# oma219/spumoni

Hardware: AMD Instinct MI355X
Metric: reads/s PML classification, 200 bp reads vs 10-hap human index (higher is better)
Workload: dtype u64

## Files before the change

### spumoni_amd/csrc/spx_cache.hip

```cpp
#include <sys/stat.h>
#include <unistd.h>
#include <algorithm>
#include <chrono>
#include <cstdio>
#include <cstring>
#include <string>
#include <thread>
#include <vector>

#include "spx_internal.h"

using namespace spx;

extern "C" {

namespace {

struct SpxFileHeader {
    char magic[8];
    char layout[56];
    uint64_t header_bytes;
    uint64_t n, r;
    uint32_t has_samples, has_docs;
    uint64_t n_text;
    uint64_t arr_bytes[spx_index::NARR];
    uint64_t arr_offset[spx_index::NARR];
    spx::DevIndex view;
    uint64_t device_bytes;
    char source_tag[128];
};

constexpr size_t STAGE = 16u << 20;

int read_to_device(FILE* f, uint64_t off, void* dst, uint64_t bytes, void* stage[2], hipStream_t st, hipEvent_t ev[2]) {
    if (fseeko(f, (off_t)off, SEEK_SET) != 0) {
        set_error("seek failed");
        return SPX_E_IO;
    }
    int b = 0;
    for (uint64_t done = 0; done < bytes; b ^= 1) {
        const size_t take = (size_t)std::min<uint64_t>(STAGE, bytes - done);
        SPX_HIP(hipEventSynchronize(ev[b]));
        if (fread(stage[b], 1, take, f) != take) {
            set_error("cache file is truncated");
            return SPX_E_IO;
        }
        SPX_HIP(hipMemcpyAsync((char*)dst + done, stage[b], take, hipMemcpyHostToDevice, st));
        SPX_HIP(hipEventRecord(ev[b], st));
        done += take;
// ... 123 lines not shown
        return SPX_E_ARG;
    }
    std::lock_guard<std::mutex> g(ix->mu);
    SPX_HIP(hipSetDevice(ix->device));
    SPX_HIP(hipDeviceSynchronize());
    SpxFileHeader h;
    memset(&h, 0, sizeof h);
    memcpy(h.magic, "SPXFLAT", 8);
    snprintf(h.layout, sizeof h.layout, "%s", SPX_LAYOUT_VERSION);
    h.header_bytes = sizeof h;
    h.n = ix->n;
    h.r = ix->r;
    h.has_samples = ix->has_samples;
    h.has_docs = ix->has_docs;
    h.n_text = ix->n_text;
    h.view = ix->view;
    {
        spx_index blank;
        blank.view = h.view;
        blank.n_text = ix->n_text;
        bind_view(&blank);
        h.view = blank.view;
    }
    h.device_bytes = ix->device_bytes;
    memcpy(h.source_tag, ix->source_tag, sizeof h.source_tag);
    uint64_t off = (sizeof h + 4095) & ~4095ull;
    for (int i = 0; i < spx_index::NARR; ++i) {
        const bool skip = i == A_FAT || i == A_FATJ;
        h.arr_bytes[i] = ix->arr_bytes[i];
        h.arr_offset[i] = skip ? 0 : off;
        if (!skip) off = (off + ix->arr_bytes[i] + 4095) & ~4095ull;
    }
    const std::string tmp = std::string(path) + ".tmp";
    FILE* f = fopen(tmp.c_str(), "wb");
    if (!f) {
        set_error("cannot create %s", tmp.c_str());
        return SPX_E_IO;
    }
    IoPool& pool = io_pool();
    std::lock_guard<std::mutex> pg(pool.mu);
    int rc = pool.init();
    if (rc == SPX_OK && (fwrite(&h, sizeof h, 1, f) != 1 || ftruncate(fileno(f), (off_t)off) != 0)) {
        set_error("write failed");
        rc = SPX_E_IO;
    }
    if (fclose(f) != 0 && rc == SPX_OK) {
        set_error("write failed (disk full?)");
        rc = SPX_E_IO;
    }
    void** arr[spx_index::NARR];
    index_arrays(ix, arr);
    for (int i = 0; i < spx_index::NARR && rc == SPX_OK; ++i)
        if (h.arr_offset[i]) rc = transfer_array(pool, tmp, h.arr_offset[i], *arr[i], h.arr_bytes[i], false, ix->device);
    if (rc == SPX_OK && rename(tmp.c_str(), path) != 0) {
        set_error("cannot rename %s to %s", tmp.c_str(), path);
        rc = SPX_E_IO;
    }
    if (rc != SPX_OK) remove(tmp.c_str());
    return rc;
}

spx_index* spx_index_load_flat(const char* path, int device) {
    if (!path) {
        set_error("path is null");
        return nullptr;
    }
    if (select_device(device) != SPX_OK) return nullptr;
    FILE* f = fopen(path, "rb");
    if (!f) {
        set_error("cannot open %s", path);
        return nullptr;
    }
    SpxFileHeader h;
    if (fread(&h, sizeof h, 1, f) != 1 || memcmp(h.magic, "SPXFLAT", 8) != 0 || h.header_bytes != sizeof h) {
        set_error("%s is not a flat-layout cache of this library", path);
        fclose(f);
        return nullptr;
    }
    h.layout[sizeof h.layout - 1] = 0;
    if (strcmp(h.layout, SPX_LAYOUT_VERSION) != 0) {
        set_error("%s was written by layout '%s', this library is '%s': rebuild the cache", path, h.layout,
                  SPX_LAYOUT_VERSION);
        fclose(f);
        return nullptr;
    }
    {
        struct stat stf;
        const uint64_t fsize = fstat(fileno(f), &stf) == 0 ? (uint64_t)stf.st_size : 0;
        const uint64_t r = h.view.r;
        const uint64_t row_bytes = h.view.compact ? sizeof(spx::Row32) : sizeof(spx::Row);
        const bool aux = h.has_samples || h.has_docs;
        uint64_t want[spx_index::NARR] = {};
        want[A_ROWS] = (r + ROW_PAD) * row_bytes;
        want[A_DIRROWS] = (r + ROW_PAD) * sizeof(spx::JumpRow);
        want[A_FAT] = (h.view.nfat + 2) * (uint64_t)h.view.fat_stride;
        want[A_FATJ] = spx::fatjs_count(h.view.nfat) * 4 + 64;
        want[A_Q] = (r + 1 + Q_PAD) * 4;
        want[A_AUX] = aux ? (r + 2) * sizeof(spx::Aux) : 0;
        want[A_SSRUN] = h.has_samples ? (r + 4) * 8 : 0;
        want[A_RUNDOCS] = h.has_docs ? (r + ROW_PAD) * 4 : 0;
        want[A_LETTERS] = 256 * sizeof(spx::LetterInfo);
        want[A_TEXT] = h.n_text ? h.n_text + 16 : 0;
        bool ok = r > 0 && r < 0xfffffff0ull && h.r > 0 && h.r <= r && h.n > 0 && h.view.n == h.n &&
                  (h.view.fat_stride == 32u || (!aux && h.view.fat_stride == 16u)) && (h.view.fat_stride == 16u || aux || h.view.compact) &&
                  (h.n_text == 0 || h.n_text + 1 == h.n || h.n_text < h.n);
        for (int i = 0; ok && i < spx_index::NARR; ++i) {
            ok = h.arr_bytes[i] == want[i];
            const bool stored = i != A_FAT && i != A_FATJ && h.arr_bytes[i] != 0;
            if (ok && stored) ok = h.arr_offset[i] >= sizeof h && h.arr_offset[i] + h.arr_bytes[i] <= fsize;
        }
        if (!ok) {
            set_error("%s: the header does not describe a consistent index (array sizes / offsets against r = %llu and the "
                      "file's %llu bytes): rebuild the cache", path, (unsigned long long)r, (unsigned long long)fsize);
            fclose(f);
            return nullptr;
        }
    }
    spx_index* ix = new spx_index();
    ix->device = device;
    h.source_tag[sizeof h.source_tag - 1] = 0;
    memcpy(ix->source_tag, h.source_tag, sizeof ix->source_tag);
    ix->n = h.n;
    ix->r = h.r;
    ix->has_samples = h.has_samples != 0;
    ix->has_docs = h.has_docs != 0;
    ix->n_text = h.n_text;
    ix->view = h.view;
    ix->device_bytes = h.device_bytes;
    const bool timing = getenv("SPX_TIMING") != nullptr;
    auto now = [] { return std::chrono::duration<double>(std::chrono::steady_clock::now().time_since_epoch()).count(); };
    auto body = [&]() -> int {
        double t0 = now();
        IoPool& pool = io_pool();
        std::lock_guard<std::mutex> pg(pool.mu);
        int rc = pool.init();
        if (rc != SPX_OK) return rc;
        if (timing) fprintf(stderr, "[spx] load_flat: staging pool %.3f s\n", now() - t0);
        void** arr[spx_index::NARR];
        index_arrays(ix, arr);
        for (int i = 0; i < spx_index::NARR; ++i) {
            ix->arr_bytes[i] = h.arr_bytes[i];
            if (h.arr_bytes[i] == 0 || h.arr_offset[i] == 0) continue;
            SPX_HIP(hipMalloc(arr[i], h.arr_bytes[i]));
            t0 = now();
            if ((rc = transfer_array(pool, path, h.arr_offset[i], *arr[i], h.arr_bytes[i], true, device)) != SPX_OK) return rc;
            if (timing) fprintf(stderr, "[spx] load_flat: array %d, %.2f GB in %.3f s\n", i, h.arr_bytes[i] / 1e9, now() - t0);
        }
        bind_view(ix);
        t0 = now();
        if ((rc = build_fat(ix)) != SPX_OK) return rc;
        if (timing) fprintf(stderr, "[spx] load_flat: fat table rebuilt in %.3f s\n", now() - t0);
        return init_runtime(ix);
    };
    const int rc = body();
    fclose(f);
    if (rc != SPX_OK) {
        spx_index_free(ix);
        return nullptr;
    }
    return ix;
}

spx_index* spx_index_clone(spx_index* src, int device) {
    if (!src) {
        set_error("index is null");
        return nullptr;
    }
    if (select_device(device) != SPX_OK) return nullptr;
    spx_index* ix = new spx_index();
    ix->device = device;
    auto body = [&]() -> int {
        std::lock_guard<std::mutex> g(src->mu);
        ix->n = src->n;
        ix->r = src->r;
// ... 44 lines not shown
        ix->force_digest_kernel = src->force_digest_kernel;
        ix->digest_parked = src->digest_parked;
        return rc;
    };
    if (body() != SPX_OK) {
        spx_index_free(ix);
        return nullptr;
    }
    return ix;
}

int spx_index_describe(const spx_index* ix, char* buf, size_t cap) {
    if (!ix || !buf || cap == 0) {
        set_error("null argument");
        return SPX_E_ARG;
    }
    const DevIndex& v = ix->view;
    char where[160] = "";
    if (getenv("SPX_DESCRIBE_ADDRESSES"))
        snprintf(where, sizeof where, ", \"rows_at\": \"%p\", \"dirrows_at\": \"%p\", \"fat_at\": \"%p\"", (void*)ix->rows, (void*)ix->dirrows, (void*)ix->fat);
    snprintf(buf, cap,
             "{\"layout\": \"%s\", \"n\": %llu, \"r\": %llu, \"flat_runs\": %u, \"letters\": %u, \"compact_rows\": %u, "
             "\"fat_slots\": %llu, \"fat_slots_per_run\": %.4f, \"fat_stride\": %u, \"has_samples\": %d, "
             "\"has_docs\": %d, \"n_text\": %llu, \"device_bytes\": %llu%s}",
             SPX_LAYOUT_VERSION, (unsigned long long)ix->n, (unsigned long long)ix->r, v.r, v.nletters, v.compact,
             (unsigned long long)v.nfat, (double)v.nfat / (double)(v.r ? v.r : 1), v.fat_stride,
             (int)ix->has_samples, (int)ix->has_docs, (unsigned long long)ix->n_text,
             (unsigned long long)(ix->device_bytes + ix->n_text), where);
    return SPX_OK;
}

}
```

### spumoni_amd/csrc/spx_flatten.hip

```cpp
#include <hipcub/hipcub.hpp>

#include <functional>

#include <algorithm>
#include <chrono>
#include <cmath>
#include <cstdio>
#include <cstdlib>
#include <vector>

#include "spx_internal.h"

namespace spx {

namespace {

constexpr int TPB = 256;
#define SPX_ALLOC0(ptr, bytes)                                   \
    do {                                                         \
        const size_t nb_ = (bytes);                              \
        SPX_HIP(hipMalloc((void**)&(ptr), nb_));                 \
        SPX_HIP(hipMemsetAsync((ptr), 0, nb_, nullptr));         \
    } while (0)
inline unsigned nblocks(uint64_t n) { return (unsigned)((n + TPB - 1) / TPB); }
// ... 277 lines not shown

__global__ void k_pack_aux(const SamplePair* samples, const uint32_t* dirdocs, uint64_t count, Aux* aux) {
    uint64_t i = blockIdx.x * (uint64_t)TPB + threadIdx.x;
    if (i >= count) return;
    const SamplePair sp = samples ? samples[i] : SamplePair{0, 0};
    aux[i] = pack_aux(sp.ss, sp.se, dirdocs ? dirdocs[i] : 0u);
}

__global__ void k_samples(const uint64_t* ssa, const uint64_t* esa, const uint32_t* Qall, uint64_t r,
                          SamplePair* out, uint64_t* ss_by_run) {
    uint64_t i = blockIdx.x * (uint64_t)TPB + threadIdx.x;
    if (i > r) return;
    SamplePair sp;
    sp.ss = i < r ? ssa[Qall[i]] : 0;
    sp.se = i > 0 ? esa[Qall[i - 1]] : 0;
    out[i] = sp;
    if (i < r) ss_by_run[i] = ssa[i];
    if (i == r) {
        ss_by_run[r] = 0;
        ss_by_run[r + 1] = 0;
    }
}

}

int build_fat(spx_index* ix) {
    hipStream_t st = nullptr;
    const uint64_t r = ix->view.r, nfat = ix->view.nfat;
    const uint32_t fat_stride = ix->view.fat_stride;
    std::vector<LetterInfo> hl(256);
    SPX_HIP(hipMemcpy(hl.data(), ix->letters, 256 * sizeof(LetterInfo), hipMemcpyDeviceToHost));
    std::vector<uint8_t> lets;
    uint64_t most_runs = 0;
    for (int c = 0; c < 256; ++c)
        if (hl[c].qend > hl[c].qbeg) {
            lets.push_back((uint8_t)c);
            most_runs = std::max<uint64_t>(most_runs, hl[c].qend - hl[c].qbeg);
            if ((hl[c].fbase & (FJ_GROUP - 1)) != 0 || hl[c].fbase + letter_slots((uint32_t)r, hl[c].bmul) > nfat) {
                set_error("index letters describe a fat table that does not fit its %llu slots", (unsigned long long)nfat);
                return SPX_E_FORMAT;
            }
        }
    if (lets.empty()) {
        set_error("index without letters");
        return SPX_E_FORMAT;
    }
// ... 468 lines not shown
    }
    if (docs) {
        SPX_HIP(hipMemcpyAsync(&last_de, d_de + (r - 1), 8, hipMemcpyDeviceToHost, st));
        SPX_HIP(hipMemcpyAsync(&first_ds, d_ds, 8, hipMemcpyDeviceToHost, st));
    }
    const bool has_ms = d_ssa && d_esa;
    SPX_HIP(hipStreamSynchronize(st));
    for (DevBuf* t : {&samples_tmp, &dirdocs_tmp, &Qall, &S, &Hs, &H, &tmp}) {
        if (t->p) (void)hipFree(t->p);
        t->p = nullptr;
    }
    if (release_inputs) release_inputs();
    size_t mem_free = 0, mem_total = 0;
    SPX_HIP(hipMemGetInfo(&mem_free, &mem_total));
    const uint32_t fat_row_bytes = sizeof(FatRow);
    const bool want_lrow = getenv("SPX_FAT_LROW") != nullptr && atoi(getenv("SPX_FAT_LROW")) != 0;
    const bool lrow = want_lrow && compact && !(has_ms || docs);
    const uint32_t fat_stride = fat_row_bytes + ((has_ms || docs || lrow) ? (uint32_t)sizeof(Aux) : 0);
    const double per_slot = fat_stride + 4.0 / FJ_GROUP ;
    const double fixed = (double)r * ((double)row_bytes + 32 + 4 + ((has_ms || docs) ? 16 : 0) + (has_ms ? 8 : 0) + (docs ? 4 : 0));
    const double to_come = (double)(64 << 20);
    double budget = 0.75 * (double)mem_total;
    if (const char* e = getenv("SPX_INDEX_BUDGET_GB")) budget = atof(e) * 1e9;
    double fat_bytes = budget - fixed;
    const double fat_bytes_free = 0.92 * (double)mem_free - to_come;
    if (fat_bytes > fat_bytes_free) fat_bytes = fat_bytes_free;
    double max_slots = fat_bytes > 0 ? fat_bytes / per_slot : 0;
    if (max_slots > 16.0 * (double)r) max_slots = 16.0 * (double)r;
    if (const char* e = getenv("SPX_FAT_SLOTS_PER_RUN")) max_slots = atof(e) * (double)r;
    double alpha = 0.7;
    if (const char* e = getenv("SPX_FAT_ALPHA")) alpha = atof(e);
    int force_bshift = -1;
    if (const char* e = getenv("SPX_FAT_BSHIFT")) {
        force_bshift = atoi(e) & 31;
        if (force_bshift > 20) force_bshift = 20;
    }
    auto geometry = [&](double K, bool commit) -> double {
        uint64_t slots = 0;
        for (uint8_t c : lets) {
            LetterInfo& li = hl[c];
            double B = force_bshift >= 0 ? (double)(1u << force_bshift)
                                         : K * pow((double)(li.qend - li.qbeg) / (double)r, -alpha);
            if (B < 1.0) B = 1.0;
            const double m = 4294967296.0 / B;
            const uint32_t bmul = m >= 4294967295.0 ? 0xffffffffu : (m < 1.0 ? 1u : (uint32_t)m);
            if (commit) {
                li.bmul = bmul;
                li.fbase = slots;
// ... 51 lines not shown
    ix->arr_bytes[A_DIRROWS] = (r + ROW_PAD) * sizeof(JumpRow);
    ix->arr_bytes[A_FAT] = (nfat + 2) * (uint64_t)fat_stride;
    ix->arr_bytes[A_FATJ] = fatjs_count(nfat) * 4 + 64;
    ix->arr_bytes[A_Q] = (r + 1 + Q_PAD) * 4;
    ix->arr_bytes[A_AUX] = ix->aux ? (r + 2) * sizeof(Aux) : 0;
    ix->arr_bytes[A_SSRUN] = ix->ss_by_run ? (r + 4) * 8 : 0;
    ix->arr_bytes[A_RUNDOCS] = ix->rundocs ? (r + ROW_PAD) * 4 : 0;
    ix->arr_bytes[A_LETTERS] = 256 * sizeof(LetterInfo);
    ix->arr_bytes[A_TEXT] = 0;
    v.n = n;
    v.r = (uint32_t)r;
    v.compact = (uint32_t)compact;
    v.nletters = nletters;
    v.nfat = nfat;
    v.init_k = (uint32_t)(r - 1);
    v.init_off = last_len - 1;
    memset(&v.init_row, 0, sizeof v.init_row);
    SPX_HIP(hipMemcpy(&v.init_row, reinterpret_cast<const char*>(ix->rows) + (r - 1) * row_bytes, row_bytes,
                      hipMemcpyDeviceToHost));
    v.init_sample = ix->has_samples ? (last_esa + 1) % n : 0;
    v.init_doc = (uint32_t)last_de;
    v.doc_at0 = (uint32_t)first_ds;
    ix->device_bytes = bytes;
    return SPX_OK;
}

}
```

### spumoni_amd/csrc/spx_internal.h

```cpp
#pragma once
#include <hip/hip_runtime.h>

#include <memory>
#include <functional>
#include <mutex>
#include <string>

#include "../../include/spumoni_gpu.h"
#include "spx_layout.h"

namespace spx {

void set_error(const char* fmt, ...);
int hip_fail(hipError_t e, const char* what, const char* file, int line);
int select_device(int device);

#define SPX_HIP(call)                                                        \
    do {                                                                     \
        hipError_t e_ = (call);                                              \
        if (e_ != hipSuccess) return spx::hip_fail(e_, #call, __FILE__, __LINE__); \
    } while (0)

struct QuietOnError {
    hipStream_t st;
// ... 75 lines not shown
    uint32_t* out_lengths;
    uint64_t* out_pointers;
    uint32_t* out_docs;
    spx_class* out_class;
    uint64_t bin_width;
    uint64_t bin_magic;
    uint64_t max_value_thr;
    WalkCounters* counters;
    uint32_t lanes_per_wave;
    uint32_t narrow;
    ChunkArgs ch;
    const uint32_t* only_flagged;
    const uint64_t* in_starts;
    uint64_t* len_mask;
    unsigned long long* claim;
    uint64_t len_mask_pairs;
};

}

namespace spx {
struct ArrayOwner {
    int device = 0;
    void* p[10] = {};
    ~ArrayOwner() {
        (void)hipSetDevice(device);
        for (void* a : p)
            if (a) (void)hipFree(a);
    }
};
}

struct spx_index {
    int device = 0;
    uint64_t n = 0, r = 0;
    bool has_samples = false, has_docs = false;
    spx::Row* rows = nullptr;
    uint32_t* q_alloc = nullptr;
    spx::JumpRow* dirrows = nullptr;
    char* fat = nullptr;
    uint32_t* fat_js = nullptr;
    spx::Aux* aux = nullptr;
    uint64_t* ss_by_run = nullptr;
    uint32_t* rundocs = nullptr;
    spx::LetterInfo* letters = nullptr;
    uint8_t* text = nullptr;
    uint64_t n_text = 0;
    static constexpr int NARR = 10;
    uint64_t arr_bytes[NARR] = {};
    std::shared_ptr<spx::ArrayOwner> owner;
    hipStream_t ctx_stream = nullptr;
    static constexpr int NDIGSCR = 15;
    hipEvent_t ev_dig = nullptr;
    hipStream_t dig_stream = nullptr;
    bool dig_used = false;
    spx::DevIndex view{};
    spx::WalkCounters* counters = nullptr;
    bool claim_used = false;
    hipEvent_t ev0 = nullptr, ev1 = nullptr, ev_done = nullptr;
    bool have_timing = false;
    hipStream_t last_stream = nullptr;
    uint64_t device_bytes = 0;
    int waves_per_cu = 0;
    int occ_blocks[8] = {};
    int num_cus = 0;
    int force_lanes_per_wave = 0;
    int force_digest_kernel = 0;
    int digest_parked = 0;
    uint8_t charhash[4] = {0, 0, 0, 0};
    char source_tag[128] = {0};
    static constexpr int PIPE_CHUNKS = 10;
// ... 41 lines not shown
           M_OUT_DOCS, M_COUNT };
    Scratch mems_scr[M_COUNT];
    hipEvent_t ev_m[4] = {nullptr, nullptr, nullptr, nullptr};
    hipStream_t mems_stream = nullptr;
    bool have_mems = false, mems_pending = false, mems_ready = false, mems_ready_docs = false;
    uint64_t mems_capacity = 0, mems_ready_n = 0;
    uint64_t mems_acc[4] = {};
    float mems_ms = 0;
    uint64_t text_bytes[3] = {0, 0, 0};
    uint64_t text_nreads = 0;
    bool text_ready = false;
    spx_class* text_cls_host = nullptr;
    int blocking_sync = 0;
    hipEvent_t ev_wait = nullptr;
    uint64_t* h_pub = nullptr;
    uint64_t* h_pub_dev = nullptr;
    int chunk_mode = 0;
    int chunk_shift = 0;
    int chunk_len = 0;
    uint64_t last_chunk_len = 0, last_chunk_bound = 0;
};

namespace spx {
enum { A_ROWS, A_DIRROWS, A_FAT, A_FATJ, A_Q, A_AUX, A_SSRUN, A_RUNDOCS, A_LETTERS, A_TEXT };
inline void index_arrays(spx_index* ix, void*** out) {
    out[A_ROWS] = (void**)&ix->rows;
    out[A_DIRROWS] = (void**)&ix->dirrows;
    out[A_FAT] = (void**)&ix->fat;
    out[A_FATJ] = (void**)&ix->fat_js;
    out[A_Q] = (void**)&ix->q_alloc;
    out[A_AUX] = (void**)&ix->aux;
    out[A_SSRUN] = (void**)&ix->ss_by_run;
    out[A_RUNDOCS] = (void**)&ix->rundocs;
    out[A_LETTERS] = (void**)&ix->letters;
    out[A_TEXT] = (void**)&ix->text;
}
inline void bind_view(spx_index* ix) {
    DevIndex& v = ix->view;
    v.rows = ix->rows;
    v.dirrows = ix->dirrows;
    v.fat = ix->fat;
    v.Q = ix->q_alloc ? ix->q_alloc + 1 : nullptr;
    v.aux = ix->aux;
    v.ss_by_run = ix->ss_by_run;
    v.rundocs = ix->rundocs;
    v.fat_js = ix->fat_js;
    v.letters = ix->letters;
    v.text = ix->text;
    v.n_text = ix->n_text;
}
int ctx_stream_of(spx_index* ix, hipStream_t* out);
int ctx_wait(spx_index* ix, hipStream_t st);
int init_runtime(spx_index* ix);
void release_votes(spx_index* ix);
void release_mems(spx_index* ix);
int build_fat(spx_index* ix);
int launch_text_check(spx_index* ix, unsigned long long* d_bad, hipStream_t stream);
int launch_text_from_index(spx_index* ix, uint8_t* d_text, uint64_t n_text, unsigned long long* d_stuck, hipStream_t stream);
int flatten_on_device(spx_index* ix, const uint8_t* d_heads, const uint64_t* d_lens,
                      const uint64_t* d_thr, const uint64_t* d_ssa, const uint64_t* d_esa,
                      const uint64_t* d_ds, const uint64_t* d_de, const std::function<void()>& release_inputs = {});
int launch_walk(spx_index* ix, int mode, const BatchArgs& args, uint64_t total_chars,
                hipStream_t stream, bool* wrote_lengths = nullptr);
int launch_ms_extend(spx_index* ix, const BatchArgs& args, hipStream_t stream);
int prepare_len_mask(spx_index* ix, int mode, BatchArgs& args);
inline uint64_t len_mask_pairs(uint64_t chars, uint64_t reads) { return (chars >> 7) + reads + 2; }
int launch_len_expand(spx_index* ix, const BatchArgs& args, hipStream_t stream);
int launch_walk_chunked(spx_index* ix, int mode, const BatchArgs& args, uint64_t total_chars, hipStream_t stream,
                        bool* done, uint64_t geom_chars = 0);
int launch_text_count(const void* d_vals, int value_bytes, const uint64_t* d_offs, const uint32_t* d_gap, uint64_t nreads,
                      uint64_t* d_line_bytes, uint64_t* d_line_start, void* d_cub, size_t cub_bytes, hipStream_t st);
size_t text_scan_bytes(uint64_t nreads);
int launch_text_write(const void* d_vals, int value_bytes, const uint64_t* d_offs, const uint32_t* d_gap, uint64_t nreads,
                      const uint64_t* d_line_start, char* d_text, hipStream_t st);
int launch_digest(spx_index* ix, int kind, uint32_t k, uint32_t w, const uint8_t* d_seqs, const uint64_t* d_offs,
                  uint64_t nreads, uint64_t total_chars, uint8_t* d_out, uint64_t* d_out_offs, hipStream_t stream,
                  bool* parked = nullptr);
}
```

### spumoni_amd/csrc/spx_layout.h

```cpp
#pragma once
#include <stdint.h>

#if defined(__HIPCC__)
#define SPX_HD __host__ __device__ __forceinline__
#else
#define SPX_HD inline
#endif

#define SPX_LAYOUT_VERSION "spx-flat-r06a"

namespace spx {

constexpr uint64_t MASK40 = (1ull << 40) - 1;
constexpr uint32_t NO_LETTER = 0xffffffffu;
constexpr int ROW_PAD = 8;
constexpr int Q_PAD = 16;

struct alignas(16) Row {
    uint64_t q0;
    uint64_t q1;
};
constexpr uint32_t ROOM_SAT = 127;

SPX_HD Row pack_row(uint32_t H, uint64_t len, uint32_t LFrun, uint64_t LFoff, bool thr_ok, uint64_t room) {
    Row r;
    const uint64_t rm = room < ROOM_SAT ? room : ROOM_SAT;
    r.q0 = (len & MASK40) | ((uint64_t)(H & 0xff) << 40) | ((uint64_t)(LFrun & 0xffff) << 48);
    r.q1 = (LFoff & MASK40) | ((uint64_t)(LFrun >> 16) << 40) | ((uint64_t)(thr_ok ? 1 : 0) << 56) | (rm << 57);
    return r;
}
SPX_HD uint32_t row_room(const Row& r) { return (uint32_t)(r.q1 >> 57); }
SPX_HD uint64_t row_len(const Row& r) { return r.q0 & MASK40; }
// ... 98 lines not shown
    uint64_t fbase;
};
SPX_HD uint32_t fat_block(uint32_t k, uint32_t bmul) { return (uint32_t)(((uint64_t)k * bmul) >> 32); }
SPX_HD uint64_t letter_slots(uint32_t r, uint32_t bmul) { return ((uint64_t)fat_block(r, bmul) + 2 + 7) & ~7ull; }

struct alignas(16) Aux {
    uint64_t a0, a1;
};
SPX_HD Aux pack_aux(uint64_t ss, uint64_t se, uint32_t docs) {
    Aux a;
    a.a0 = (ss & MASK40) | ((se & 0xffffff) << 40);
    a.a1 = ((se >> 24) & 0xffff) | ((uint64_t)docs << 16);
    return a;
}
SPX_HD uint64_t aux_ss(const Aux& a) { return a.a0 & MASK40; }
SPX_HD uint64_t aux_se(const Aux& a) { return (a.a0 >> 40) | ((a.a1 & 0xffff) << 24); }
SPX_HD uint32_t aux_docs(const Aux& a) { return (uint32_t)(a.a1 >> 16); }

struct SamplePair {
    uint64_t ss;
    uint64_t se;
};

struct DevIndex {
    const Row* rows;
    const JumpRow* dirrows;
    const char* fat;
    const uint32_t* Q;
    const Aux* aux;
    const uint64_t* ss_by_run;
    const uint32_t* rundocs;
    const uint32_t* fat_js;
    uint32_t fat_stride;
    const LetterInfo* letters;
    const uint8_t* text;
    uint64_t n_text;
    uint64_t n;
    uint32_t r;
    uint32_t compact;
    uint32_t nletters;
    uint64_t nfat;
    uint32_t init_k;
    uint64_t init_off;
    Row32 init_row;
    uint64_t init_sample;
    uint32_t init_doc;
    uint32_t doc_at0;
};

SPX_HD const Row& row_at(const DevIndex& ix, uint64_t k) {
    return *reinterpret_cast<const Row*>(reinterpret_cast<const char*>(ix.rows) + k * (ix.compact ? sizeof(Row32) : sizeof(Row)));
}

constexpr uint64_t PIECE_MAX = 65535;

SPX_HD uint64_t run_of_position(const uint64_t* S, uint64_t r, uint64_t p) {
    uint64_t lo = 0, hi = r;
    while (hi - lo > 1) {
        const uint64_t mid = lo + (hi - lo) / 2;
        if (S[mid] <= p)
            lo = mid;
        else
            hi = mid;
    }
    return lo;
}

template <class F>
SPX_HD uint32_t for_each_piece(uint64_t len, uint64_t lf, const uint64_t* S, uint64_t a, uint64_t nb, uint32_t span, F&& f) {
    uint32_t np = 0;
// ... 19 lines not shown
```

### spumoni_amd/csrc/spx_walk_fast.inc

```

enum : uint32_t { Q_LAND = 0, Q_FAT = 1, Q_STEP = 2, Q_READ = 3, Q_CHARS = 4, Q_FATJ = 5, Q_QS = 6, Q_DIR = 7, Q_DONE = 8, Q_SAMP = 9, Q_START = 10, Q_WANT = 11 };
enum : uint32_t {
    F_EMB = 1,
    F_NOROW = 2,
    F_QUIRK = 4,
    F_WIDE = 16,
    F_FADD = 32,
    F_HAVEC = 64,
    F_SAMPD = 128
};
enum : uint32_t { A_STEP = 1, A_EMIT = 2, A_DECIDE = 4 };
#ifndef SPX_STEP_REPS
#define SPX_STEP_REPS 2
#endif
constexpr int STEP_REPS = SPX_STEP_REPS;
constexpr uint32_t OFF_LAST32 = 0xffffffffu;
#ifndef SPX_CHUNK_CLAIM
#define SPX_CHUNK_CLAIM 64
#endif
constexpr uint32_t CHUNK_CLAIM = SPX_CHUNK_CLAIM;
static_assert(CHUNK_CLAIM >= 64, "a claim covers at least one iteration's worst case: 64 lanes ending a read each");

__device__ __forceinline__ uint32_t dpp_swap1(uint32_t v) { return (uint32_t)__builtin_amdgcn_mov_dpp((int)v, 0xB1, 0xf, 0xf, true); }

struct alignas(16) HotLetter {
    uint32_t bmul;
    uint32_t present;
    uint64_t fat0;
};

__device__ __forceinline__ void lf_target_ct(uint32_t LFrun, uint32_t LFoff, uint32_t cums, uint32_t off, uint32_t& k0,
                                             uint32_t& offp, uint32_t& t_out) {
    lf_target_c(LFrun, LFoff, cums, off, k0, offp);
    const uint32_t t = k0 - LFrun;
    t_out = (t < 4 && off <= 126) ? t : 4u;
}

template <int MODE, bool DOC, bool NARROW, int CHUNK = 0, bool EARLY = false, bool DYN = false>
__global__ void __launch_bounds__(WALK_TPB) k_walk_fast(const DevIndex ix, const BatchArgs b) {
    constexpr bool AUX = (MODE == SPX_MODE_MS) || DOC;
    constexpr bool PML = MODE == SPX_MODE_PML;
    if (CHUNK == 2 && b.ch.round > 1 && b.ch.pending[b.ch.round] == 0) return;
    __shared__ HotLetter s_hot[256];
#ifndef SPX_PGRP
#define SPX_PGRP 16
#endif
    constexpr int PGRP = SPX_PGRP, PROW = WALK_TPB + 1;
    constexpr int PLPG = PGRP / 2, PNG = 64 / PLPG;
    __shared__ uint64_t s_ptrs[MODE == SPX_MODE_MS && CHUNK != 2 ? PGRP * PROW : 1];
    constexpr bool DSTAGE = PML && DOC && CHUNK != 2;
    constexpr int DGRP = 32, DROW = DGRP + 2;
    __shared__ uint16_t s_docs[DSTAGE ? WALK_TPB * DROW : 1];
    const LetterInfo* const s_let = ix.letters;
    __shared__ uint32_t s_win[8 * WALK_TPB];
    const char* const rows_b = reinterpret_cast<const char*>(ix.rows);
    const char* const fat_b = reinterpret_cast<const char*>(ix.fat);
    const uint32_t fs = ix.fat_stride;
    const bool lrow = !AUX && fs == 32 && ix.aux == nullptr;
    for (int t = threadIdx.x; t < 256; t += blockDim.x) {
        const LetterInfo li = ix.letters[t];
        s_hot[t] = HotLetter{li.bmul, li.qbeg != li.qend ? 1u : 0u, (uint64_t)(uintptr_t)(fat_b + li.fbase * fs)};
    }
    __syncthreads();
    const char* const dir_b = reinterpret_cast<const char*>(ix.dirrows);
    const char* const fatj_b = reinterpret_cast<const char*>(ix.fat_js);
    const char* const q_b = reinterpret_cast<const char*>(ix.Q);
    const char* const seq_b = reinterpret_cast<const char*>(b.seqs);
    const char* const off_b = reinterpret_cast<const char*>(b.offs);
    const uint32_t R = ix.r;
    const uint32_t fs_shift = fs == 32 ? 5 : 4;
    const bool want_class = PML && CHUNK == 0 && b.out_class != nullptr;
    const bool want_len = PML && CHUNK != 2 && b.out_lengths != nullptr;
    const uint32_t lpw = b.lanes_per_wave;
    const uint32_t nlanes = (uint32_t)((((uint64_t)gridDim.x * blockDim.x) >> 6) * lpw);
    const uint32_t nitems = CHUNK ? (uint32_t)*b.ch.nchunks : (uint32_t)b.nreads;
    const uint64_t ch_org = CHUNK ? b.offs[0] : 0;
    uint8_t* const ch_flags = CHUNK ? b.ch.flags - (ch_org & ~7ull) : nullptr;
    WalkState* const ch_ckpt = CHUNK ? b.ch.ckpt - (ch_org >> CKPT_SHIFT) : nullptr;
    const char* const item_b = CHUNK ? reinterpret_cast<const char*>(b.ch.desc) : off_b;
    constexpr uint32_t ITEM_BYTES = CHUNK ? sizeof(ChunkDesc) : 8;
    const uint32_t tid = threadIdx.x;
    static_assert(!DYN || (CHUNK == 0 && !EARLY), "only the plain, full launch deals its reads on demand");
    uint32_t w_n0 = 0, w_e0 = 0, w_n1 = 0, w_e1 = 0;
    bool w_pend = false;
// ... 65 lines not shown
                const u32x4 t = *(GV16)(uintptr_t)a2;
                r2x = t.x, r2y = t.y, r2z = t.z, r2w = t.w;
            }
            ga = V16{odd ? r2x : r1x, odd ? r2y : r1y, odd ? r2z : r1z, odd ? r2w : r1w};
            const uint32_t zx = dpp_swap1(odd ? r1x : r2x), zy = dpp_swap1(odd ? r1y : r2y), zz = dpp_swap1(odd ? r1z : r2z),
                           zw = dpp_swap1(odd ? r1w : r2w);
            gb = V16{w_own ? zx : 0u, w_own ? zy : 0u, w_own ? zz : 0u, w_own ? zw : 0u};
        }
        side_doc = 0;
        side_aux = Aux{0, 0};
        side_in = 0;
        claimed = 0;
        if (CHUNK == 0 && b.in_starts != nullptr && ph == Q_READ) side_in = b.in_starts[rd];
        if (DOC && ph == Q_SAMP) side_doc = ix.rundocs[k];
        if (AUX && ph == Q_DIR) side_aux = ix.aux[length];
        if (DYN && w_pend && (tid & 63) == 0) claimed = atomicAdd(b.claim, (unsigned long long)CHUNK_CLAIM);
    };
    if (EARLY) issue_gather();
    while (__builtin_amdgcn_ballot_w64(ph != Q_DONE) != 0) {
        if (!EARLY) issue_gather();
        uint32_t act = 0, hd = 0;
        uint32_t rflag = 0;
        bool pred_ev = false;
        uint32_t d_trun = 0, d_toff = 0, d_srun = 0, d_soff = 0, d_bits = 0;
        Aux d_aux{0, 0};
        bool d_lrow = false;
        uint64_t fbits = 0;
        uint32_t fxi = 0;
        bool flush = false;
        bool pflush = false, pheld = false, pheld_end = false;
        uint32_t pfxi = 0;
        uint64_t phold = 0;
        COUNT(w_rows, ph == Q_LAND);
        COUNT(w_dir, ph == Q_FAT || (ph >= Q_FATJ && ph <= Q_DIR));

        if (ph == Q_LAND) {
            const uint32_t len = ga.x & 0xffffu;
            const uint32_t o = off == OFF_LAST32 ? len - 1 : off;
            if (o >= len) {
                off = o - len;
                k++;
                addr += sizeof(Row32);
            } else {
                off = o;
                q0 = u64of(ga.x, ga.y);
                q1 = u64of(ga.z, ga.w);
                fl = (fl & ~F_NOROW) | F_EMB;
                act = A_STEP;
            }
        } else if (ph == Q_FAT) {
            const uint32_t hq = ga.x;
            const uint32_t w1l = ga.z, w1h = ga.w;
            const bool nosucc = (w1h >> 29) & 1, esc = (w1h >> 30) & 1;
            const bool quirk = fl & F_QUIRK;
            const bool found = nosucc || hq > k || (quirk && hq == k);
            if (found && !esc && !quirk) {
                d_trun = hq - (w1l & 0x7ffffu);
// ... 63 lines not shown
                        bin_lo = (nb - 1) * w;
                        bin_max = above = below = 0;
                        sum_max = 0;
                    }
                    act = A_STEP;
                    if (CHUNK == 2) {
                        ph = Q_START;
                        addr = reinterpret_cast<const char*>(b.ch.round > 1 ? b.ch.reentry + rd : b.ch.ends + rd + 1);
                        fl = F_WIDE;
                        act = 0;
                    }
                }
            } else if (ph == Q_CHARS) {
                s_win[0 * WALK_TPB + tid] = ga.x;
                s_win[1 * WALK_TPB + tid] = ga.y;
                s_win[2 * WALK_TPB + tid] = ga.z;
                s_win[3 * WALK_TPB + tid] = ga.w;
                s_win[4 * WALK_TPB + tid] = gb.x;
                s_win[5 * WALK_TPB + tid] = gb.y;
                s_win[6 * WALK_TPB + tid] = gb.z;
                s_win[7 * WALK_TPB + tid] = gb.w;
                ph = Q_STEP;
                act = A_STEP;
            } else if (CHUNK == 2 && ph == Q_START) {
                k = ga.x;
                length = ga.y;
                {
                    const uint64_t offp = u64of(ga.z, ga.w);
                    off = offp == OFF_END ? OFF_LAST32 : (uint32_t)offp;
                }
                sample = u64of(gb.x, gb.y);
                doc = gb.z;
                tlimit = b.ch.round > 1 ? gb.w : 0xffffffffu;
                ph = Q_LAND;
                addr = rows_b + (uint64_t)k * sizeof(Row32);
                fl = F_WIDE;
                {
                    const char* const cp = reinterpret_cast<const char*>(ch_ckpt + ((base + m - 1) >> CKPT_SHIFT));
                    cka = *reinterpret_cast<const V16*>(cp);
                    ckb = *reinterpret_cast<const V16*>(cp + 16);
                }
            } else if (ph == Q_FATJ) {
                const uint32_t lo = (length & 2) ? ga.z : ga.x, hi = (length & 2) ? ga.w : ga.y;
                length = (length & 1) ? hi : lo;
                fl |= F_WIDE;
                ph = Q_QS;
// ... 36 lines not shown
                    if (AUX) {
                        const Aux a = ix.aux[jdir + ((below_thr && off > 0) ? 1u : 0u)];
                        if (MODE == SPX_MODE_MS) sample = below_thr ? aux_se(a) : aux_ss(a);
                        if (DOC) doc = below_thr ? (aux_docs(a) >> 16) : (aux_docs(a) & 0xffffu);
                    }
                    if (!below_thr) {
                        k = LFrun_k;
                        off = LFoff_k + off;
                    } else if (off > 0) {
                        k = LFrun_k;
                        off = LFoff_k + off - 1;
                    } else {
                        if (jdir <= qbeg) atomicAdd(&b.counters->error, 1ull);
                        const bool ps = jr_psame(e);
                        const uint32_t srun = jr_sLFrun(e);
                        k = ps ? srun : srun - 1;
                        off = ps ? (uint32_t)jr_sLFoff(e) - 1 : OFF_LAST32;
                    }
                    length = 0;
                    fl &= ~(F_EMB | F_QUIRK);
                    rflag = 3;
                    act = A_EMIT;
                }
            }
        }
        if (AUX && ph == Q_SAMP) {
            if (MODE == SPX_MODE_MS) sample = u64of(ga.x, ga.y);
            if (DOC) doc = side_doc & 0xffffu;
            fl |= F_SAMPD;
            ph = Q_STEP;
            act = A_STEP;
        }

        {
            const bool dec = act & A_DECIDE;
            const bool nosucc = (d_bits >> 9) & 1, psame = (d_bits >> 8) & 1;
            const bool below_thr = nosucc || (k < d_trun) || (k == d_trun && off < d_toff);
            COUNT(w_pred, (dec && below_thr) || pred_ev);
            if (dec) {
                if (below_thr && ((d_bits >> 10) & 1)) atomicAdd(&b.counters->error, 1ull);
                const bool last = below_thr && !psame;
                k = d_srun - (last ? 1u : 0u);
                off = last ? OFF_LAST32 : d_soff - (below_thr ? 1u : 0u);
                hd = last ? ((d_bits >> 16) & 0xffu) : (d_bits & 0xffu);
                if (MODE == SPX_MODE_MS) sample = below_thr ? aux_se(d_aux) : aux_ss(d_aux);
                if (DOC) doc = below_thr ? (aux_docs(d_aux) >> 16) : (aux_docs(d_aux) & 0xffffu);
// ... 437 lines not shown
```

Before: 1.098 billion.

## Add precomputed start table to skip first backward-search steps per read

Builds a device table of walk states for every string of the first `depth` letters, filled level by level with a GPU kernel. When a read's last `depth` characters are all present letters, the PML walk fetches one table entry and replays the stored reset bits into the match-length and bin statistics, instead of doing `depth` LF/jump steps. The table is sized against the memory budget and takes space from the fat table. It is rebuilt at cache load rather than stored in the file, which bumps the layout version. Saving is at most a few steps out of roughly 200 per read, and the new phase adds a dependent load plus extra branching and ballots in the hot loop.

```diff
diff --git a/spumoni_amd/csrc/spx_cache.hip b/spumoni_amd/csrc/spx_cache.hip
--- a/spumoni_amd/csrc/spx_cache.hip
+++ b/spumoni_amd/csrc/spx_cache.hip
@@ -23,8 +23,8 @@
     uint64_t n, r;
     uint32_t has_samples, has_docs;
     uint64_t n_text;
-    uint64_t arr_bytes[spx_index::NARR];
-    uint64_t arr_offset[spx_index::NARR];
+    uint64_t arr_bytes[spx_index::NFILE];
+    uint64_t arr_offset[spx_index::NFILE];
     spx::DevIndex view;
     uint64_t device_bytes;
     char source_tag[128];
@@ -194,10 +194,10 @@
         bind_view(&blank);
         h.view = blank.view;
     }
-    h.device_bytes = ix->device_bytes;
+    h.device_bytes = ix->device_bytes - ix->arr_bytes[A_START];
     memcpy(h.source_tag, ix->source_tag, sizeof h.source_tag);
     uint64_t off = (sizeof h + 4095) & ~4095ull;
-    for (int i = 0; i < spx_index::NARR; ++i) {
+    for (int i = 0; i < spx_index::NFILE; ++i) {
         const bool skip = i == A_FAT || i == A_FATJ;
         h.arr_bytes[i] = ix->arr_bytes[i];
         h.arr_offset[i] = skip ? 0 : off;
@@ -222,7 +222,7 @@
     }
     void** arr[spx_index::NARR];
     index_arrays(ix, arr);
-    for (int i = 0; i < spx_index::NARR && rc == SPX_OK; ++i)
+    for (int i = 0; i < spx_index::NFILE && rc == SPX_OK; ++i)
         if (h.arr_offset[i]) rc = transfer_array(pool, tmp, h.arr_offset[i], *arr[i], h.arr_bytes[i], false, ix->device);
     if (rc == SPX_OK && rename(tmp.c_str(), path) != 0) {
         set_error("cannot rename %s to %s", tmp.c_str(), path);
@@ -262,7 +262,7 @@
         const uint64_t r = h.view.r;
         const uint64_t row_bytes = h.view.compact ? sizeof(spx::Row32) : sizeof(spx::Row);
         const bool aux = h.has_samples || h.has_docs;
-        uint64_t want[spx_index::NARR] = {};
+        uint64_t want[spx_index::NFILE] = {};
         want[A_ROWS] = (r + ROW_PAD) * row_bytes;
         want[A_DIRROWS] = (r + ROW_PAD) * sizeof(spx::JumpRow);
         want[A_FAT] = (h.view.nfat + 2) * (uint64_t)h.view.fat_stride;
@@ -276,7 +276,7 @@
         bool ok = r > 0 && r < 0xfffffff0ull && h.r > 0 && h.r <= r && h.n > 0 && h.view.n == h.n &&
                   (h.view.fat_stride == 32u || (!aux && h.view.fat_stride == 16u)) && (h.view.fat_stride == 16u || aux || h.view.compact) &&
                   (h.n_text == 0 || h.n_text + 1 == h.n || h.n_text < h.n);
-        for (int i = 0; ok && i < spx_index::NARR; ++i) {
+        for (int i = 0; ok && i < spx_index::NFILE; ++i) {
             ok = h.arr_bytes[i] == want[i];
             const bool stored = i != A_FAT && i != A_FATJ && h.arr_bytes[i] != 0;
             if (ok && stored) ok = h.arr_offset[i] >= sizeof h && h.arr_offset[i] + h.arr_bytes[i] <= fsize;
@@ -310,7 +310,7 @@
         if (timing) fprintf(stderr, "[spx] load_flat: staging pool %.3f s\n", now() - t0);
         void** arr[spx_index::NARR];
         index_arrays(ix, arr);
-        for (int i = 0; i < spx_index::NARR; ++i) {
+        for (int i = 0; i < spx_index::NFILE; ++i) {
             ix->arr_bytes[i] = h.arr_bytes[i];
             if (h.arr_bytes[i] == 0 || h.arr_offset[i] == 0) continue;
             SPX_HIP(hipMalloc(arr[i], h.arr_bytes[i]));
@@ -322,6 +322,11 @@
         t0 = now();
         if ((rc = build_fat(ix)) != SPX_OK) return rc;
         if (timing) fprintf(stderr, "[spx] load_flat: fat table rebuilt in %.3f s\n", now() - t0);
+        t0 = now();
+        const int depth = getenv("SPX_START_DEPTH") ? start_depth_for(h.view.nletters, (int)h.view.compact, h.device_bytes)
+                                                    : (int)h.view.start_depth;
+        if ((rc = build_start(ix, depth)) != SPX_OK) return rc;
+        if (timing) fprintf(stderr, "[spx] load_flat: start table (depth %u) rebuilt in %.3f s\n", ix->view.start_depth, now() - t0);
         return init_runtime(ix);
     };
     const int rc = body();
@@ -412,10 +417,11 @@
     snprintf(buf, cap,
              "{\"layout\": \"%s\", \"n\": %llu, \"r\": %llu, \"flat_runs\": %u, \"letters\": %u, \"compact_rows\": %u, "
              "\"fat_slots\": %llu, \"fat_slots_per_run\": %.4f, \"fat_stride\": %u, \"has_samples\": %d, "
-             "\"has_docs\": %d, \"n_text\": %llu, \"device_bytes\": %llu%s}",
+             "\"has_docs\": %d, \"n_text\": %llu, \"start_depth\": %u, \"start_bytes\": %llu, \"device_bytes\": %llu%s}",
              SPX_LAYOUT_VERSION, (unsigned long long)ix->n, (unsigned long long)ix->r, v.r, v.nletters, v.compact,
              (unsigned long long)v.nfat, (double)v.nfat / (double)(v.r ? v.r : 1), v.fat_stride,
-             (int)ix->has_samples, (int)ix->has_docs, (unsigned long long)ix->n_text,
+             (int)ix->has_samples, (int)ix->has_docs, (unsigned long long)ix->n_text, v.start_depth,
+             (unsigned long long)ix->arr_bytes[A_START],
              (unsigned long long)(ix->device_bytes + ix->n_text), where);
     return SPX_OK;
 }
diff --git a/spumoni_amd/csrc/spx_flatten.hip b/spumoni_amd/csrc/spx_flatten.hip
--- a/spumoni_amd/csrc/spx_flatten.hip
+++ b/spumoni_amd/csrc/spx_flatten.hip
@@ -323,6 +323,157 @@
     }
 }
 
+__device__ bool start_step(const DevIndex& ix, uint32_t c, uint32_t& k, uint32_t& off, uint32_t& length, uint32_t& jumps,
+                           uint32_t& pred) {
+    const Row32* rows = reinterpret_cast<const Row32*>(ix.rows);
+    const uint32_t R = ix.r;
+    const Row row{rows[k].q0, rows[k].q1};
+    const LetterInfo li = ix.letters[c];
+    const bool eq = k < R && crow_H(row) == c;
+    const bool lf = eq && (c < 128 || crow_thr_ok(row));
+    uint32_t nk = 0, noff = 0;
+    bool last = false;
+    if (lf) {
+        nk = crow_LFrun(row);
+        noff = crow_LFoff(row) + off;
+        if (c < 128) {
+            length++;
+        } else {
+            length = 0;
+            jumps++;
+        }
+    } else {
+        jumps++;
+        length = 0;
+        uint32_t lo = li.qbeg, hi = li.qend;
+        while (lo < hi) {
+            const uint32_t mid = lo + ((hi - lo) >> 1);
+            if (ix.Q[mid] < k)
+                lo = mid + 1;
+            else
+                hi = mid;
+        }
+        const uint32_t j = lo;
+        const JumpRow e = ix.dirrows[j];
+        const uint32_t trun = jr_THRrun(e), srun = jr_sLFrun(e);
+        const uint64_t toff = jr_THRoff(e);
+        bool stay = false, back = false;
+        if (!eq) {
+            back = j >= li.qend || k < trun || (k == trun && off < toff);
+        } else {
+            const bool below = k < trun || (k == trun && off < toff);
+            stay = !below || off > 0;
+            back = below && off == 0;
+            pred += below ? 1u : 0u;
+            nk = crow_LFrun(row);
+            noff = crow_LFoff(row) + off - (below ? 1u : 0u);
+        }
+        if (!stay) {
+            if (back && j <= li.qbeg) return false;
+            if (!eq) pred += back ? 1u : 0u;
+            last = back && !jr_psame(e);
+            nk = srun - (last ? 1u : 0u);
+            noff = last ? 0u : (uint32_t)jr_sLFoff(e) - (back ? 1u : 0u);
+        }
+    }
+    if (last) {
+        noff = crow_len(Row{rows[nk].q0, rows[nk].q1}) - 1;
+    } else {
+        for (uint32_t len = crow_len(Row{rows[nk].q0, rows[nk].q1}); nk < R && noff >= len; len = crow_len(Row{rows[nk].q0, rows[nk].q1})) {
+            noff -= len;
+            nk++;
+        }
+    }
+    k = nk;
+    off = noff;
+    return true;
+}
+
+__global__ void k_start_level(const DevIndex ix, const uint8_t* lets, uint32_t nletters, const StartEntry* prev, StartEntry* out,
+                              uint64_t count) {
+    const uint64_t i = blockIdx.x * (uint64_t)TPB + threadIdx.x;
+    if (i >= count) return;
+    const uint32_t c = lets[i % nletters];
+    uint32_t k = ix.init_k, off = (uint32_t)ix.init_off, length = 0, jumps = 0, pred = 0, resets = 0;
+    bool valid = true;
+    if (prev) {
+        const StartEntry p = prev[i / nletters];
+        valid = (uint32_t)p.meta & START_VALID;
+        k = p.k;
+        off = p.off;
+        length = (uint32_t)p.meta & 0xffu;
+        jumps = ((uint32_t)p.meta >> 8) & 0xffu;
+        pred = ((uint32_t)p.meta >> 16) & 0xffu;
+        resets = (uint32_t)(p.meta >> 32);
+    }
+    StartEntry e{0, 0, 0, 0, 0};
+    if (valid && start_step(ix, c, k, off, length, jumps, pred)) {
+        const Row32* rows = reinterpret_cast<const Row32*>(ix.rows);
+        resets = (resets << 1) | (length == 0 ? 1u : 0u);
+        e.q0 = rows[k].q0;
+        e.q1 = rows[k].q1;
+        e.k = k;
+        e.off = off;
+        e.meta = (uint64_t)(length | (jumps << 8) | (pred << 16) | START_VALID) | ((uint64_t)resets << 32);
+    }
+    out[i] = e;
+}
+
+}
+
+int start_depth_for(uint32_t nletters, int compact, uint64_t index_bytes) {
+    if (!compact || nletters == 0) return 0;
+    if (const char* e = getenv("SPX_START_DEPTH")) {
+        int d = atoi(e) < 0 ? 0 : (atoi(e) > START_MAX_DEPTH ? START_MAX_DEPTH : atoi(e));
+        while (d > 0 && start_entries(nletters, d, START_FORCED_BYTES) == 0) --d;
+        return d;
+    }
+    const uint64_t cap = std::min<uint64_t>(START_MAX_BYTES, index_bytes / 64);
+    int d = 0;
+    while (d < START_MAX_DEPTH && start_entries(nletters, d + 1, cap) != 0) ++d;
+    return d;
+}
+
+int build_start(spx_index* ix, int depth) {
+    hipStream_t st = nullptr;
+    if (ix->start) (void)hipFree(ix->start);
+    ix->start = nullptr;
+    ix->device_bytes -= ix->arr_bytes[A_START];
+    ix->arr_bytes[A_START] = 0;
+    ix->view.start_depth = 0;
+    std::vector<LetterInfo> hl(256);
+    SPX_HIP(hipMemcpy(hl.data(), ix->letters, 256 * sizeof(LetterInfo), hipMemcpyDeviceToHost));
+    std::vector<uint8_t> lets;
+    for (int w = 0; w < 4; ++w) ix->view.letter_mask[w] = 0;
+    for (int c = 0; c < 256; ++c)
+        if (hl[c].qend > hl[c].qbeg) {
+            lets.push_back((uint8_t)c);
+            ix->view.letter_mask[c >> 6] |= 1ull << (c & 63);
+        }
+    const uint32_t nl = (uint32_t)lets.size();
+    const uint64_t entries = ix->view.compact ? start_entries(nl, depth, START_FORCED_BYTES) : 0;
+    bind_view(ix);
+    if (entries == 0) return SPX_OK;
+    DevBuf dl, tmp;
+    SPX_HIP(dl.alloc(256));
+    SPX_HIP(hipMemcpyAsync(dl.p, lets.data(), lets.size(), hipMemcpyHostToDevice, st));
+    SPX_HIP(hipMalloc((void**)&ix->start, entries * sizeof(StartEntry)));
+    if (depth > 1) SPX_HIP(tmp.alloc(entries / nl * sizeof(StartEntry)));
+    const StartEntry* prev = nullptr;
+    uint64_t count = 1;
+    for (int level = 1; level <= depth; ++level) {
+        count *= nl;
+        StartEntry* out = ((depth - level) & 1) ? tmp.as<StartEntry>() : ix->start;
+        k_start_level<<<nblocks(count), TPB, 0, st>>>(ix->view, dl.as<uint8_t>(), nl, prev, out, count);
+        prev = out;
+    }
+    SPX_HIP(hipGetLastError());
+    SPX_HIP(hipStreamSynchronize(st));
+    ix->arr_bytes[A_START] = entries * sizeof(StartEntry);
+    ix->device_bytes += ix->arr_bytes[A_START];
+    ix->view.start_depth = (uint32_t)depth;
+    bind_view(ix);
+    return SPX_OK;
 }
 
 int build_fat(spx_index* ix) {
@@ -837,8 +988,12 @@
     const double to_come = (double)(64 << 20);
     double budget = 0.75 * (double)mem_total;
     if (const char* e = getenv("SPX_INDEX_BUDGET_GB")) budget = atof(e) * 1e9;
-    double fat_bytes = budget - fixed;
-    const double fat_bytes_free = 0.92 * (double)mem_free - to_come;
+    double planned = budget - fixed < 0.92 * (double)mem_free - to_come ? budget - fixed : 0.92 * (double)mem_free - to_come;
+    if (planned > 16.0 * (double)r * per_slot) planned = 16.0 * (double)r * per_slot;
+    const int start_depth = start_depth_for(nletters, compact, (uint64_t)(fixed + (planned > 0 ? planned : 0)));
+    const double start_bytes = (double)(start_entries(nletters, start_depth, START_FORCED_BYTES) * sizeof(StartEntry));
+    double fat_bytes = budget - fixed - start_bytes;
+    const double fat_bytes_free = 0.92 * (double)mem_free - to_come - start_bytes * (start_depth > 1 ? 1.0 + 1.0 / nletters : 1.0);
     if (fat_bytes > fat_bytes_free) fat_bytes = fat_bytes_free;
     double max_slots = fat_bytes > 0 ? fat_bytes / per_slot : 0;
     if (max_slots > 16.0 * (double)r) max_slots = 16.0 * (double)r;
@@ -936,7 +1091,7 @@
     v.init_doc = (uint32_t)last_de;
     v.doc_at0 = (uint32_t)first_ds;
     ix->device_bytes = bytes;
-    return SPX_OK;
-}
-
-}
+    return build_start(ix, start_depth);
+}
+
+}
diff --git a/spumoni_amd/csrc/spx_internal.h b/spumoni_amd/csrc/spx_internal.h
--- a/spumoni_amd/csrc/spx_internal.h
+++ b/spumoni_amd/csrc/spx_internal.h
@@ -121,7 +121,7 @@
 namespace spx {
 struct ArrayOwner {
     int device = 0;
-    void* p[10] = {};
+    void* p[11] = {};
     ~ArrayOwner() {
         (void)hipSetDevice(device);
         for (void* a : p)
@@ -145,7 +145,9 @@
     spx::LetterInfo* letters = nullptr;
     uint8_t* text = nullptr;
     uint64_t n_text = 0;
-    static constexpr int NARR = 10;
+    spx::StartEntry* start = nullptr;
+    static constexpr int NARR = 11;
+    static constexpr int NFILE = 10;
     uint64_t arr_bytes[NARR] = {};
     std::shared_ptr<spx::ArrayOwner> owner;
     hipStream_t ctx_stream = nullptr;
@@ -233,7 +235,7 @@
 };
 
 namespace spx {
-enum { A_ROWS, A_DIRROWS, A_FAT, A_FATJ, A_Q, A_AUX, A_SSRUN, A_RUNDOCS, A_LETTERS, A_TEXT };
+enum { A_ROWS, A_DIRROWS, A_FAT, A_FATJ, A_Q, A_AUX, A_SSRUN, A_RUNDOCS, A_LETTERS, A_TEXT, A_START };
 inline void index_arrays(spx_index* ix, void*** out) {
     out[A_ROWS] = (void**)&ix->rows;
     out[A_DIRROWS] = (void**)&ix->dirrows;
@@ -245,6 +247,7 @@
     out[A_RUNDOCS] = (void**)&ix->rundocs;
     out[A_LETTERS] = (void**)&ix->letters;
     out[A_TEXT] = (void**)&ix->text;
+    out[A_START] = (void**)&ix->start;
 }
 inline void bind_view(spx_index* ix) {
     DevIndex& v = ix->view;
@@ -259,6 +262,7 @@
     v.letters = ix->letters;
     v.text = ix->text;
     v.n_text = ix->n_text;
+    v.start = ix->start;
 }
 int ctx_stream_of(spx_index* ix, hipStream_t* out);
 int ctx_wait(spx_index* ix, hipStream_t st);
@@ -266,6 +270,8 @@
 void release_votes(spx_index* ix);
 void release_mems(spx_index* ix);
 int build_fat(spx_index* ix);
+int start_depth_for(uint32_t nletters, int compact, uint64_t index_bytes);
+int build_start(spx_index* ix, int depth);
 int launch_text_check(spx_index* ix, unsigned long long* d_bad, hipStream_t stream);
 int launch_text_from_index(spx_index* ix, uint8_t* d_text, uint64_t n_text, unsigned long long* d_stuck, hipStream_t stream);
 int flatten_on_device(spx_index* ix, const uint8_t* d_heads, const uint64_t* d_lens,
diff --git a/spumoni_amd/csrc/spx_layout.h b/spumoni_amd/csrc/spx_layout.h
--- a/spumoni_amd/csrc/spx_layout.h
+++ b/spumoni_amd/csrc/spx_layout.h
@@ -7,7 +7,7 @@
 #define SPX_HD inline
 #endif
 
-#define SPX_LAYOUT_VERSION "spx-flat-r06a"
+#define SPX_LAYOUT_VERSION "spx-flat-r07a"
 
 namespace spx {
 
@@ -152,6 +152,24 @@
     uint64_t se;
 };
 
+struct alignas(32) StartEntry {
+    uint64_t q0, q1;
+    uint32_t k, off;
+    uint64_t meta;
+};
+constexpr uint32_t START_VALID = 1u << 31;
+constexpr int START_MAX_DEPTH = 12;
+constexpr uint64_t START_MAX_BYTES = 512ull << 20;
+constexpr uint64_t START_FORCED_BYTES = 8ull << 30;
+SPX_HD uint64_t start_entries(uint32_t nletters, int d, uint64_t max_bytes) {
+    uint64_t e = 1;
+    for (int i = 0; i < d; ++i) {
+        e *= nletters;
+        if (e * sizeof(StartEntry) > max_bytes) return 0;
+    }
+    return d > 0 && nletters > 0 ? e : 0;
+}
+
 struct DevIndex {
     const Row* rows;
     const JumpRow* dirrows;
@@ -176,6 +194,9 @@
     uint64_t init_sample;
     uint32_t init_doc;
     uint32_t doc_at0;
+    const StartEntry* start;
+    uint32_t start_depth;
+    uint64_t letter_mask[4];
 };
 
 SPX_HD const Row& row_at(const DevIndex& ix, uint64_t k) {
diff --git a/spumoni_amd/csrc/spx_walk_fast.inc b/spumoni_amd/csrc/spx_walk_fast.inc
--- a/spumoni_amd/csrc/spx_walk_fast.inc
+++ b/spumoni_amd/csrc/spx_walk_fast.inc
@@ -1,5 +1,5 @@
 
-enum : uint32_t { Q_LAND = 0, Q_FAT = 1, Q_STEP = 2, Q_READ = 3, Q_CHARS = 4, Q_FATJ = 5, Q_QS = 6, Q_DIR = 7, Q_DONE = 8, Q_SAMP = 9, Q_START = 10, Q_WANT = 11 };
+enum : uint32_t { Q_LAND = 0, Q_FAT = 1, Q_STEP = 2, Q_READ = 3, Q_CHARS = 4, Q_FATJ = 5, Q_QS = 6, Q_DIR = 7, Q_DONE = 8, Q_SAMP = 9, Q_START = 10, Q_WANT = 11, Q_TAB = 12 };
 enum : uint32_t {
     F_EMB = 1,
     F_NOROW = 2,
@@ -20,6 +20,7 @@
 #endif
 constexpr uint32_t CHUNK_CLAIM = SPX_CHUNK_CLAIM;
 static_assert(CHUNK_CLAIM >= 64, "a claim covers at least one iteration's worst case: 64 lanes ending a read each");
+static_assert(START_MAX_DEPTH + STEP_REPS <= 64, "the emits of a start-table entry and of the repetitions after it complete at most one word of reset bits");
 
 __device__ __forceinline__ uint32_t dpp_swap1(uint32_t v) { return (uint32_t)__builtin_amdgcn_mov_dpp((int)v, 0xB1, 0xf, 0xf, true); }
 
@@ -57,9 +58,17 @@
     const char* const fat_b = reinterpret_cast<const char*>(ix.fat);
     const uint32_t fs = ix.fat_stride;
     const bool lrow = !AUX && fs == 32 && ix.aux == nullptr;
+    constexpr bool TAB = PML && !DOC && CHUNK == 0;
+    const uint32_t tab_d = (TAB && ix.start != nullptr) ? ix.start_depth : 0u;
+    const uint32_t tab_nl = ix.nletters;
+    const char* const tab_b = reinterpret_cast<const char*>(ix.start);
     for (int t = threadIdx.x; t < 256; t += blockDim.x) {
         const LetterInfo li = ix.letters[t];
-        s_hot[t] = HotLetter{li.bmul, li.qbeg != li.qend ? 1u : 0u, (uint64_t)(uintptr_t)(fat_b + li.fbase * fs)};
+        uint32_t rank = 0;
+#pragma unroll
+        for (int w = 0; w < 4; ++w)
+            rank += (uint32_t)__popcll(ix.letter_mask[w] & (t >= 64 * (w + 1) ? ~0ull : (t > 64 * w ? (1ull << (t - 64 * w)) - 1 : 0ull)));
+        s_hot[t] = HotLetter{li.bmul, li.qbeg != li.qend ? rank + 1 : 0u, (uint64_t)(uintptr_t)(fat_b + li.fbase * fs)};
     }
     __syncthreads();
     const char* const dir_b = reinterpret_cast<const char*>(ix.dirrows);
@@ -171,6 +180,7 @@
         uint32_t act = 0, hd = 0;
         uint32_t rflag = 0;
         bool pred_ev = false;
+        uint32_t tab_meta = 0;
         uint32_t d_trun = 0, d_toff = 0, d_srun = 0, d_soff = 0, d_bits = 0;
         Aux d_aux{0, 0};
         bool d_lrow = false;
@@ -181,7 +191,7 @@
         uint32_t pfxi = 0;
         uint64_t phold = 0;
         COUNT(w_rows, ph == Q_LAND);
-        COUNT(w_dir, ph == Q_FAT || (ph >= Q_FATJ && ph <= Q_DIR));
+        COUNT(w_dir, ph == Q_FAT || (ph >= Q_FATJ && ph <= Q_DIR) || (TAB && ph == Q_TAB));
 
         if (ph == Q_LAND) {
             const uint32_t len = ga.x & 0xffffu;
@@ -291,6 +301,62 @@
                 s_win[7 * WALK_TPB + tid] = gb.w;
                 ph = Q_STEP;
                 act = A_STEP;
+                if (TAB && tab_d != 0 && x == m && m > tab_d) {
+                    uint32_t idx = 0;
+                    bool all = true;
+                    for (uint32_t i = 0; i < tab_d; ++i) {
+                        const uint32_t rk = s_hot[WIN_AT(wi - (int32_t)i)].present;
+                        all = all && rk != 0;
+                        idx = idx * tab_nl + rk - 1;
+                    }
+                    if (all) {
+                        ph = Q_TAB;
+                        addr = tab_b + (uint64_t)idx * sizeof(StartEntry);
+                        fl = F_WIDE;
+                        act = 0;
+                    }
+                }
+            } else if (TAB && ph == Q_TAB) {
+                ph = Q_STEP;
+                act = A_STEP;
+                fl = 0;
+                const uint32_t meta = gb.z;
+                if (meta & START_VALID) {
+                    q0 = u64of(ga.x, ga.y);
+                    q1 = u64of(ga.z, ga.w);
+                    k = gb.x;
+                    off = gb.y;
+                    uint32_t rs = gb.w << (32 - tab_d);
+                    uint32_t len = 0;
+                    for (uint32_t i = 0; i < tab_d; ++i) {
+                        const uint32_t xi = x - 1;
+                        x = xi;
+                        const uint32_t reset = rs >> 31;
+                        rs <<= 1;
+                        len = reset ? 0u : len + 1;
+                        mbits = (mbits << 1) | reset;
+                        if ((xi & 63) == 0) {
+                            fbits = mbits;
+                            fxi = xi;
+                            flush = true;
+                            mbits = 0;
+                        }
+                        if (want_class) {
+                            if (xi < bin_lo) {
+                                const bool ab = bin_max >= b.max_value_thr;
+                                above += ab ? 1u : 0u;
+                                below += ab ? 0u : 1u;
+                                sum_max += bin_max;
+                                bin_max = 0;
+                                bin_lo -= (uint32_t)b.bin_width;
+                            }
+                            bin_max = len > bin_max ? len : bin_max;
+                        }
+                    }
+                    length = len;
+                    wi -= (int32_t)tab_d;
+                    tab_meta = meta;
+                }
             } else if (CHUNK == 2 && ph == Q_START) {
                 k = ga.x;
                 length = ga.y;
@@ -373,6 +439,13 @@
                     rflag = 3;
                     act = A_EMIT;
                 }
+            }
+        }
+        if (TAB && __builtin_amdgcn_ballot_w64(tab_meta != 0) != 0) {
+#pragma unroll
+            for (int bit = 0; bit < 4; ++bit) {
+                w_jumps += (uint32_t)__popcll(__builtin_amdgcn_ballot_w64((tab_meta >> (8 + bit)) & 1)) << bit;
+                w_pred += (uint32_t)__popcll(__builtin_amdgcn_ballot_w64((tab_meta >> (16 + bit)) & 1)) << bit;
             }
         }
         if (AUX && ph == Q_SAMP) {
```

Result: slower. 1.042 billion (-5.2%).
